# wangjunchi/LLMSeg

Hardware: AMD Instinct MI355X
Metric: images/sec (1024x1024, 64-tok prompt) model_forward fwd+bwd (higher is better)
Workload: dtype bf16; 1 GPU; BASELINE.json configs[2]: synthetic 1024x1024 + random-init LLaVA-7B(Llama-7B+CLIP-L/14)/SAM-ViT-H, batch_size=2 per GPU, fwd+bwd train step (CE + align + IoP losses, LoRA r=8 dropout 0.05 on q/v + trainable embed/lm_head/text_fcs/lisa_*, frozen towers, fp32 gradient arena, AdamW step every 10 micro-steps inside the timed region, micro-step replayed from a hipGraph), 256 candidate masks, 64-token ; global_batch=2, parallelism=dp1, graph=True, valid=True

## Files before the change

include/llmseg_hip.h:

```cpp
#ifndef LLMSEG_HIP_H
#define LLMSEG_HIP_H

#include <stdint.h>

#ifdef __cplusplus
extern "C" {
#endif

#define LLMSEG_OK 0
#define LLMSEG_EINVAL (-1)
#define LLMSEG_ELAUNCH (-2)
#define LLMSEG_NOT_TAKEN 1

enum { LLMSEG_ACT_NONE = 0, LLMSEG_ACT_RELU = 1, LLMSEG_ACT_GELU = 2, LLMSEG_ACT_QUICKGELU = 3, LLMSEG_ACT_SILU = 4,
       LLMSEG_ACT_SIGMOID = 5 };

#define LLMSEG_ABI_VERSION 11

#define LLMSEG_REDUCE_WS_BYTES (16 << 20)
int llmseg_version(void);
int64_t llmseg_launch_count(void);
int64_t llmseg_struct_size(int which);
const char* llmseg_last_error(void);

typedef struct {
  uint32_t struct_size;
  uint32_t reserved0;
  const void* A; const void* W; void* C;
  const void* bias;
  const void* gamma;
  const void* residual;
  int64_t M, N, K;
  int64_t lda, ldw, ldc, ldr;
  int64_t batch, strideA, strideW, strideC;
  float alpha;
  int act;
  int out_f32;
  int trans_a;
  int trans_w;
  int64_t batch2, strideA2, strideW2, strideC2;
// ... 137 lines not shown
int llmseg_intersection_union(const uint8_t* pred, const uint8_t* target, int64_t n, int32_t ignore_index, int64_t* out, void* stream);

int llmseg_union_resize_iou(const uint8_t* segs, const uint8_t* select, const uint8_t* gt, int32_t H, int32_t W, int32_t K, int32_t Hg, int32_t Wg,
                            int32_t out_h, int32_t out_w, int32_t ignore_index, int64_t* out, void* stream);

int llmseg_gt_resample(const uint8_t* gt, const int32_t* gy, const int32_t* gx, uint8_t* out, int32_t H, int32_t W, int32_t Hg, int32_t Wg, void* stream);
int llmseg_proposal_targets(const uint8_t* masks, const int64_t* order, const uint8_t* gtp, int32_t n_gt, void* out, int32_t K, int32_t H, int32_t W,
                            int32_t out_size, const int32_t* y0, const int32_t* ny, const double* wy, const int32_t* x0, const int32_t* nx,
                            const double* wx, int32_t taps, int64_t* counts, int64_t* gt_area, double* iou, double* iop, void* stream);
int llmseg_rle_decode(const uint32_t* run_ends, const int64_t* offsets, uint8_t* out, int32_t K, int32_t H, int32_t W, int32_t hwk, void* stream);
int llmseg_mask_targets(const uint8_t* segs, const uint8_t* gt, const int32_t* gy, const int32_t* gx, int32_t K, int32_t H, int32_t W, int32_t Hg,
                        int32_t Wg, int64_t* counts, int64_t* gt_area, double* iou, double* iop, void* stream);
int llmseg_resize_aa(const uint8_t* segs, void* out, int32_t K, int32_t H, int32_t W, int32_t out_size, const int32_t* y0, const int32_t* ny,
                     const double* wy, const int32_t* x0, const int32_t* nx, const double* wx, int32_t taps, void* stream);

int llmseg_colsum(const void* x, float* out, int64_t M, int64_t N, int64_t ld, void* workspace, int64_t workspace_bytes, void* stream);
int llmseg_norm_bwd(const void* dy, const void* x, const void* w, void* dx, float* dw, float* db, int64_t rows, int64_t cols,
                    float eps, int rms, void* workspace, int64_t workspace_bytes, void* stream);
int llmseg_norm_bwd_add(const void* dy, const void* x, const void* w, const void* dres, void* dx, float* dw, float* db, int64_t rows, int64_t cols,
                        float eps, int rms, void* workspace, int64_t workspace_bytes, void* stream);
int llmseg_swiglu_bwd(const void* gu, const void* dout, void* dgu, int64_t rows, int64_t I, void* stream);
int llmseg_act_bwd(const void* dy, const void* y, void* out, int64_t n, int act, void* stream);
int llmseg_linear_bwd(const void* dy, const void* y, int act, const void* x, const void* w, void* dx, float* dw, float* db, int64_t M, int64_t N, int64_t K,
                      int accumulate, void* stream);
int llmseg_softmax_rows(const float* S, void* P, int64_t BH, int32_t Tq, int32_t Tk, int32_t ld, float scale, int32_t causal,
                        const uint8_t* key_mask, int32_t heads, void* stream);
int llmseg_attn_ds(const void* P, const float* dP, void* dS, int64_t rows, int32_t T, int32_t ld, float scale, void* stream);
int llmseg_ce_bwd(const void* logits, const int64_t* labels, const float* coef, void* dlogits, int32_t N, int32_t T, int64_t V,
                  int64_t ldl, void* stream);
int llmseg_scatter_add_rows(const void* src, const int64_t* idx, float* dst, int64_t n, int64_t cols, void* stream);
typedef struct {
  const uint64_t* rng_state;
  uint32_t stream;
  uint32_t drop_thr;
  uint32_t seg_rows;
  uint32_t reserved0;
} llmseg_dropout;
int llmseg_lora_down(const void* x0, const void* x1, int64_t ldx, const void* w0, const void* w1, void* y, int64_t ldy, int64_t M, int64_t K,
                     int32_t w_kr, float alpha, int32_t zero_cols, const llmseg_dropout* drop, void* stream);
int llmseg_lora_down_ws(const void* x0, const void* x1, int64_t ldx, const void* w0, const void* w1, void* y, int64_t ldy, int64_t M, int64_t K,
                        int32_t w_kr, float alpha, int32_t zero_cols, const llmseg_dropout* drop, void* scratch, int64_t scratch_bytes, void* stream);
int llmseg_lora_outer(const void* a0, const void* a1, int64_t lda, const void* b0, const void* b1, int64_t ldb, float* out0, float* out1, int64_t M,
                      int64_t N, int32_t out_rn, float alpha, const llmseg_dropout* drop, void* workspace, int64_t workspace_bytes, void* stream);
int llmseg_lora_wgrads(const void* dq, const void* dv, int64_t ldd, const void* x, int64_t ldx, const void* xa, int64_t ldxa, const void* t, int64_t ldt,
                       float* gbq, float* gbv, float* gaq, float* gav, int64_t M, int64_t H, float s, const llmseg_dropout* drop, void* workspace,
                       int64_t workspace_bytes, void* stream);
int llmseg_lora_apply(void* y, int64_t ldy, const void* xa, int64_t ldxa, const void* w0, const void* w1, int64_t M, int64_t N, int32_t w_rn,
// ... 24 lines not shown
```

llmseg_amd/_lib.py:

```python
import ctypes as C
import os

_HERE = os.path.dirname(os.path.abspath(__file__))
LIB_PATH = os.environ.get("LLMSEG_LIB") or os.path.join(_HERE, "libllmseg_hip.so")

ABI_VERSION = 11

ACT_NONE, ACT_RELU, ACT_GELU, ACT_QUICKGELU, ACT_SILU, ACT_SIGMOID = range(6)
NOT_TAKEN = 1


class _Sized(C.Structure):

    def __init__(self, *a, **kw):
        super().__init__(*a, **kw)
        self.struct_size = C.sizeof(self)


class GemmArgs(_Sized):
    _fields_ = [("struct_size", C.c_uint32), ("reserved0", C.c_uint32), ("A", C.c_void_p), ("W", C.c_void_p), ("C", C.c_void_p),
                ("bias", C.c_void_p), ("gamma", C.c_void_p), ("residual", C.c_void_p),
                ("M", C.c_int64), ("N", C.c_int64), ("K", C.c_int64),
                ("lda", C.c_int64), ("ldw", C.c_int64), ("ldc", C.c_int64), ("ldr", C.c_int64),
                ("batch", C.c_int64), ("strideA", C.c_int64), ("strideW", C.c_int64), ("strideC", C.c_int64),
                ("alpha", C.c_float), ("act", C.c_int), ("out_f32", C.c_int), ("trans_a", C.c_int), ("trans_w", C.c_int),
                ("batch2", C.c_int64), ("strideA2", C.c_int64), ("strideW2", C.c_int64), ("strideC2", C.c_int64),
                ("A2", C.c_void_p), ("W2", C.c_void_p), ("lda2", C.c_int64), ("ldw2", C.c_int64),
                ("workspace", C.c_void_p), ("workspace_bytes", C.c_int64), ("accumulate", C.c_int),
                ("a_norm_w", C.c_void_p), ("a_norm_eps", C.c_float), ("a_swiglu", C.c_int),
# ... 77 lines not shown
    "llmseg_mask_pullback": [_p, _p, _p, _p, _i32, _i32, _i32, _p],
    "llmseg_upsample_maskpool": [_p, _p, _p, _p, _p, _p, _i32, _i32, _i32, _i32, _p],
    "llmseg_cosine_scores": [_p, _p, _p, _i32, _i32, _p],
    "llmseg_linear_f32": [_p, _i64, _p, _i64, _i32, _p, _p, _i64, _p, _i64, _i32, _i32, _i32, _i32, _f32, _p],
    "llmseg_layernorm_f32": [_p, _p, _p, _p, _i64, _i32, _f32, _p],
    "llmseg_attn_f32": [_p, _p, _p, _p, C.POINTER(C.c_int64), _i32, _i32, _i32, _i32, _i32, _f32, _p],
    "llmseg_cosine_f32": [_p, _p, _p, _i32, _i32, _p],
    "llmseg_align_reg_loss": [_p, _p, _p, _p, _p, _p, _p, _p, _p, _i32, _i32, _f32, _i32, _p],
    "llmseg_dice_bce": [_p, _p, _p, _i32, _i64, _f32, _p, _i64, _p],
    "llmseg_dice_bce_bwd": [_p, _p, _p, _p, _i32, _i64, _f32, _p],
    "llmseg_ce_loss": [_p, _p, _p, _i32, _i32, _i64, _i64, _p, _i64, _p],
    "llmseg_intersection_union": [_p, _p, _i64, _i32, _p, _p],
    "llmseg_union_resize_iou": [_p, _p, _p, _i32, _i32, _i32, _i32, _i32, _i32, _i32, _i32, _p, _p],
    "llmseg_rle_decode": [_p, _p, _p, _i32, _i32, _i32, _i32, _p],
    "llmseg_mask_targets": [_p, _p, _p, _p, _i32, _i32, _i32, _i32, _i32, _p, _p, _p, _p, _p],
    "llmseg_gt_resample": [_p, _p, _p, _p, _i32, _i32, _i32, _i32, _p],
    "llmseg_proposal_targets": [_p, _p, _p, _i32, _p, _i32, _i32, _i32, _i32, _p, _p, _p, _p, _p, _p, _i32, _p, _p, _p, _p, _p],
    "llmseg_resize_aa": [_p, _p, _i32, _i32, _i32, _i32, _p, _p, _p, _p, _p, _p, _i32, _p],
    "llmseg_colsum": [_p, _p, _i64, _i64, _i64, _p, _i64, _p],
    "llmseg_norm_bwd": [_p, _p, _p, _p, _p, _p, _i64, _i64, _f32, C.c_int, _p, _i64, _p],
    "llmseg_norm_bwd_add": [_p, _p, _p, _p, _p, _p, _p, _i64, _i64, _f32, C.c_int, _p, _i64, _p],
    "llmseg_swiglu_bwd": [_p, _p, _p, _i64, _i64, _p],
    "llmseg_act_bwd": [_p, _p, _p, _i64, C.c_int, _p],
    "llmseg_linear_bwd": [_p, _p, C.c_int, _p, _p, _p, _p, _p, _i64, _i64, _i64, C.c_int, _p],
    "llmseg_softmax_rows": [_p, _p, _i64, _i32, _i32, _i32, _f32, _i32, _p, _i32, _p],
    "llmseg_attn_ds": [_p, _p, _p, _i64, _i32, _i32, _f32, _p],
    "llmseg_ce_bwd": [_p, _p, _p, _p, _i32, _i32, _i64, _i64, _p],
    "llmseg_scatter_add_rows": [_p, _p, _p, _i64, _i64, _p],
    "llmseg_lora_down": [_p, _p, _i64, _p, _p, _p, _i64, _i64, _i64, _i32, _f32, _i32, _dp, _p],
    "llmseg_lora_down_ws": [_p, _p, _i64, _p, _p, _p, _i64, _i64, _i64, _i32, _f32, _i32, _dp, _p, _i64, _p],
    "llmseg_lora_outer": [_p, _p, _i64, _p, _p, _i64, _p, _p, _i64, _i64, _i32, _f32, _dp, _p, _i64, _p],
    "llmseg_lora_wgrads": [_p, _p, _i64, _p, _i64, _p, _i64, _p, _i64, _p, _p, _p, _p, _i64, _i64, _f32, _dp, _p, _i64, _p],
    "llmseg_lora_apply": [_p, _i64, _p, _i64, _p, _p, _i64, _i64, _i32, _f32, _dp, _p],
    "llmseg_lora_pack": [_p, _p, _p, _p, _p, _p, _p, _i64, _f32, _p],
    "llmseg_lora_down_parts": [_p, _p, _i64, _p, _p, _p, _i64, _i64, _i64, _i32, _f32, _i32, _dp, _p, _i64, C.POINTER(C.c_int32), C.POINTER(C.c_float), _p],
    "llmseg_lora_down_pack": [_p, _p, _i64, _p, _p, _p, _i64, _i64, _i64, _i32, _f32, _i32, _dp, _p, _i64, _p, _p, _p, _p, _p, _p, _p, _i64, _f32, _p],
    "llmseg_transpose_pad": [_p, _p, _i64, _i64, _i64, _i64, _i64, _p],
    "llmseg_sumsq": [_p, _i64, C.c_int, _p, _p, _i64, _p],
    "llmseg_adamw": [_p, _p, _p, C.c_int, _p, _p, _i64, _f32, _f32, _f32, _f32, _f32, _i64, _p, _p],
    "llmseg_prof_enable": [C.c_int],
    "llmseg_prof_dominant_kernel": [],
    "llmseg_prof_dominant_bytes": [],
    "llmseg_prof_dominant_info": [C.POINTER(C.c_int64)],
    "llmseg_prof_collect": [C.POINTER(C.c_double), C.POINTER(C.c_double), C.POINTER(C.c_int64), C.POINTER(C.c_double), C.POINTER(C.c_double),
                            C.POINTER(C.c_int64)],
}

# ... 30 lines not shown
```

llmseg_amd/autograd.py:

```python
import math
import os

import torch
from torch.autograd import Function

from . import ops

BF16 = torch.bfloat16


BIG_LINEAR = 1 << 34
BIG_WEIGHT = 1 << 26
FUSE_ROPE_BWD = os.environ.get("LLMSEG_NO_FUSE_ROPE_BWD") is None
FUSE_ROPE_FWD = os.environ.get("LLMSEG_NO_FUSE_ROPE_FWD") is None
FUSE_NORM_BWD = os.environ.get("LLMSEG_NO_FUSE_NORM_BWD") is None
FUSE_LORA_PARTS = os.environ.get("LLMSEG_NO_FUSE_LORA_PARTS") is None
FUSE_DELTA = os.environ.get("LLMSEG_NO_FUSE_DELTA") is None
FUSE_MLP = os.environ.get("LLMSEG_NO_FUSE_MLP") is None
FUSE_LINEAR_BWD = os.environ.get("LLMSEG_NO_FUSE_LINEAR_BWD") is None


class Leaves:
    on = False
    _streams = {}
    _keep = []
    _used = False

    @classmethod
    def run(cls, fn, *operands):
        if not cls.on:
            return fn()
        cur = torch.cuda.current_stream()
        key = cur.device.index
        side = cls._streams.get(key)
        if side is None:
            side = cls._streams[key] = torch.cuda.Stream(device=cur.device)
        side.wait_stream(cur)
        with torch.cuda.stream(side):
            out = fn()
        cls._keep.extend(operands)
        cls._used = True
        return out
# ... 26 lines not shown
    def forward(ctx, x, w, b, act, residual, wt=None):
        y = ops.gemm(x, w, bias=b, act=act, residual=residual)
        ctx.wt = wt
        ctx.act = act
        ctx.has_res = residual is not None
        ctx.gw, ctx.gb = g32_of(w), (g32_of(b) if b is not None else None)
        ctx.b_needs = b is not None and b.requires_grad
        assert not (act != ops.ACT_NONE and residual is not None)
        assert act in (ops.ACT_NONE, ops.ACT_RELU, ops.ACT_SIGMOID), "only relu/sigmoid epilogues are differentiated"
        ctx.save_for_backward(x, w, y if act != ops.ACT_NONE else None)
        return y

    @staticmethod
    def backward(ctx, dy):
        x, w, y = ctx.saved_tensors
        dy = dy.contiguous()
        N = w.shape[0]
        M, Kin = x.shape
        dx = dw = db = None
        gw = ctx.gw
        need_w = gw is not None or ctx.needs_input_grad[1]
        big = M * N * Kin >= BIG_LINEAR or (N * Kin >= BIG_WEIGHT and M >= 16)
        dres = dy if (ctx.has_res and ctx.needs_input_grad[4]) else None
        if FUSE_LINEAR_BWD and not Leaves.on and not (big and Kin % 8 == 0) and not (ctx.wt is not None and N % 8 == 0):
            need_b = ctx.gb is not None or (ctx.b_needs and ctx.needs_input_grad[2])
            acc = gw is not None or ctx.gb is not None
            new = torch.zeros if acc else torch.empty
            fw = gw if gw is not None else (new((N, Kin), device=x.device, dtype=torch.float32) if need_w else None)
            fb = ctx.gb if ctx.gb is not None else (new((N,), device=x.device, dtype=torch.float32) if need_b else None)
            if ctx.needs_input_grad[0] or fw is not None or fb is not None:
                r = ops.linear_bwd(dy, y, ctx.act, x.contiguous(), w.contiguous(), want_dx=ctx.needs_input_grad[0], dw=fw, db=fb, accumulate=acc)
                if not isinstance(r, str):
                    return (r, fw.to(BF16) if (gw is None and need_w) else None, fb.to(BF16) if (ctx.gb is None and need_b) else None, None, dres, None)
        dpre = ops.act_bwd(dy, y, ctx.act) if ctx.act != ops.ACT_NONE else dy
        if big and Kin % 8 == 0 and (need_w or ctx.wt is None or N % 8 != 0):
            Np, Mp = (N + 63) // 64 * 64, (M + 63) // 64 * 64
            if Np != N:
                dpp = torch.zeros((M, Np), device=dpre.device, dtype=BF16)
                dpp[:, :N] = dpre
            else:
                dpp = dpre
            if ctx.needs_input_grad[0]:
                dx = ops.gemm(dpp, ops.transpose_pad(w, Np))
            if need_w:
                if gw is not None:
                    def wgrad():
                        dT, xT = ops.transpose_pad(dpp, Mp), ops.transpose_pad(x, Mp)
                        ops.gemm(dT[:N], xT, out=gw, accumulate=True)
                    Leaves.run(wgrad, dpp, x)
                else:
                    dT, xT = ops.transpose_pad(dpp, Mp), ops.transpose_pad(x, Mp)
                    dw = ops.gemm(dT, xT)[:N]
        else:
            if N % 8 != 0:
                dpre_p = _pad8_cols(dpre)
                w_p = torch.zeros((dpre_p.shape[1], w.shape[1]), device=w.device, dtype=w.dtype)
                w_p[:N] = w
            else:
                dpre_p, w_p = dpre, w
            if ctx.needs_input_grad[0]:
                dx = ops.gemm(dpre, ctx.wt) if (ctx.wt is not None and N % 8 == 0) else ops.gemm(dpre_p, w_p, trans_w=True)
            if gw is not None:
                Leaves.run(lambda: ops.gemm(dpre_p[:, :N], x, out=gw, trans_a=True, trans_w=True, accumulate=True), dpre_p, x)
            elif need_w:
                dw = ops.gemm(dpre_p, x, trans_a=True, trans_w=True)[:N]
                if dw.shape[0] != N or not dw.is_contiguous():
                    dw = dw.contiguous()
        if ctx.gb is not None:
            Leaves.run(lambda: ops.colsum(dpre, out=ctx.gb), dpre)
        elif ctx.b_needs and ctx.needs_input_grad[2]:
            db = ops.colsum(dpre).to(BF16)
        return dx, dw, db, None, dres, None


def linear(x, w, b=None, act=ops.ACT_NONE, residual=None, wt=None):
    return LinearFn.apply(x, w, b, act, residual, wt)


class LinearNormFn(Function):

    @staticmethod
    def forward(ctx, x, w, b, act, residual, wt, norm_w, eps):
        assert b is None and act == ops.ACT_NONE and residual is not None
        h = torch.empty((x.shape[0], w.shape[0]), device=x.device, dtype=BF16)
        y = ops.gemm(x, w, residual=residual, norm_w=norm_w, norm_eps=eps, norm_out=h)
        ctx.wt, ctx.act, ctx.has_res = wt, act, True
        ctx.gw, ctx.gb, ctx.b_needs = g32_of(w), None, False
        ctx.save_for_backward(x, w, None)
        ctx.mark_non_differentiable(h)
        ctx.set_materialize_grads(False)
        return y, h

    @staticmethod
    def backward(ctx, dy, _dh):
        return LinearFn.backward(ctx, dy) + (None, None)


def linear_norm(x, w, residual, wt, norm_w, eps):
    return LinearNormFn.apply(x, w, None, ops.ACT_NONE, residual, wt, norm_w, eps)
# ... 557 lines not shown
```

llmseg_amd/csrc/backward.hip:

```cpp
#include <algorithm>
#include <cstdlib>
#include "common.h"
#include "llmseg_hip.h"

namespace {

inline unsigned grid_for(long total) {
  long g = (total + 255) / 256;
  return (unsigned)(g < 1 ? 1 : (g > 8192 ? 8192 : g));
}

__global__ __launch_bounds__(256) void colsum_kernel(const bf16_t* __restrict__ x, float* __restrict__ out, float* __restrict__ part, long M, long N, long ld) {
  __shared__ float red[4][64];
  const int c = threadIdx.x & 63, rl = threadIdx.x >> 6;
  const long col = (long)blockIdx.x * 64 + c;
  const long rows_per = (M + gridDim.y - 1) / gridDim.y;
  const long r0 = (long)blockIdx.y * rows_per, r1 = min(M, r0 + rows_per);
  float s = 0.f;
  if (col < N)
    for (long r = r0 + rl; r < r1; r += 4) s += bf2f(x[r * ld + col]);
  red[rl][c] = s;
  __syncthreads();
  if (rl == 0 && col < N) {
    const float v = (red[0][c] + red[1][c]) + (red[2][c] + red[3][c]);
// ... 1174 lines not shown
  const int rc = llmseg_lora_down_ws(x0, x1, ldx, w0, w1, y, ldy, M, K, w_kr, alpha, zero_cols, drop, scratch, scratch_bytes, stream);
  const bool done = g_pack_req.done;
  g_pack_req.active = false;
  if (rc != LLMSEG_OK || done) return rc;
  return llmseg_lora_pack(aq, bq, av, bv, w2b, w2a, bt, H, s, stream);
}

extern "C" int llmseg_transpose_pad(const void* in, void* out, int64_t rows, int64_t cols, int64_t ld_in, int64_t ld_out, int64_t rows_pad, void* stream) {
  LL_CHECK(in && out && rows > 0 && cols > 0 && rows_pad >= rows && ld_out >= rows_pad && ld_in >= cols, "transpose_pad: bad arguments");
  LL_CHECK((cols & 7) == 0 && (ld_in & 7) == 0 && (ld_out & 7) == 0 && (rows_pad & 7) == 0 && AL16(in) && AL16(out),
           "transpose_pad: cols, rows_pad and leading dimensions must be multiples of 8, pointers 16-byte aligned");
  LL_LAUNCH_KERNEL(transpose_pad_kernel, dim3((unsigned)((cols + 63) / 64), (unsigned)((rows_pad + 63) / 64)), dim3(256), 0, (hipStream_t)stream,
                     (const bf16_t*)in, (bf16_t*)out, (long)rows, (long)cols, (long)ld_in, (long)ld_out, (long)rows_pad);
  LL_LAUNCH_CHECK("transpose_pad");
  return LLMSEG_OK;
}

namespace {
constexpr int LB_TI = 32, LB_TK = 64, LB_CC = 256, LB_LD = LB_CC + 8;

struct LinBwd {
  const bf16_t *dy, *y, *x, *w;
  bf16_t* dx;
  float *dw, *db;
  int M, N, K, act, accumulate;
  int w_it, w_kt, x_kt;
  int vec_n, vec_k;
};

__device__ __forceinline__ uint4 lb_load8(const bf16_t* __restrict__ p, int r, int c, int rows, int cols, bool vec) {
  if (r >= rows || c >= cols) return make_uint4(0, 0, 0, 0);
  const bf16_t* q = p + (long)r * cols + c;
  if (vec) return *reinterpret_cast<const uint4*>(q);
  uint32_t h[8];
#pragma unroll
  for (int j = 0; j < 8; ++j) h[j] = c + j < cols ? (uint32_t)q[j] : 0u;
  return make_uint4(h[0] | (h[1] << 16), h[2] | (h[3] << 16), h[4] | (h[5] << 16), h[6] | (h[7] << 16));
}

__device__ __forceinline__ uint4 lb_act8(const uint4& g, const uint4& yv, int act) {
  if (act == LLMSEG_ACT_NONE) return g;
  float gf[8], yf[8];
  uint32_t o[8];
  unpack8(g, gf); unpack8(yv, yf);
#pragma unroll
  for (int e = 0; e < 8; ++e) o[e] = f2bf(act == LLMSEG_ACT_RELU ? (yf[e] > 0.f ? gf[e] : 0.f) : gf[e] * yf[e] * (1.f - yf[e]));
  return make_uint4(o[0] | (o[1] << 16), o[2] | (o[3] << 16), o[4] | (o[5] << 16), o[6] | (o[7] << 16));
}

__device__ __forceinline__ uint32_t lb_elem(const uint4& v, int j) {
  const uint32_t wd = (j >> 1) == 0 ? v.x : (j >> 1) == 1 ? v.y : (j >> 1) == 2 ? v.z : v.w;
  return (j & 1) ? (wd >> 16) : (wd & 0xffffu);
}

__device__ __forceinline__ void lb_store_t(bf16_t* T, int col0, int c, const uint4& lo, const uint4& hi) {
#pragma unroll
  for (int j = 0; j < 8; ++j) *reinterpret_cast<uint32_t*>(T + (col0 + j) * LB_LD + c) = lb_elem(lo, j) | (lb_elem(hi, j) << 16);
}

__global__ __launch_bounds__(256) void linear_bwd_kernel(const LinBwd p) {
  __shared__ __attribute__((aligned(16))) bf16_t lds[(LB_TI + LB_TK) * LB_LD];
  bf16_t* AT = lds;
  bf16_t* BT = lds + LB_TI * LB_LD;
  const int t = threadIdx.x, lane = t & 63, wave = t >> 6;
  const int nW = p.w_it * p.w_kt;
  const bool roleW = (int)blockIdx.x < nW;
  const int bi = roleW ? (int)blockIdx.x : (int)blockIdx.x - nW;
  const int nkt = roleW ? p.w_kt : p.x_kt;
  const int i0 = (bi / nkt) * LB_TI, k0 = (bi % nkt) * LB_TK;
  const int C = roleW ? p.M : p.N;
  const bf16_t* __restrict__ B = roleW ? p.x : p.w;
  const bool vn = p.vec_n != 0, vk = p.vec_k != 0, has_act = p.act != LLMSEG_ACT_NONE;
  const bool want_db = roleW && (bi % nkt) == 0 && p.db != nullptr;

  uint4 ra[4], ry[4], rb[8];
  auto load_chunk = [&](int c0) {
#pragma unroll
    for (int q = 0; q < 4; ++q) {
      int r, c;
      if (roleW) { const int pr = t + 256 * (q >> 1); r = c0 + 2 * (pr >> 2) + (q & 1); c = i0 + 8 * (pr & 3); }
      else { const int v = t + 256 * q; r = i0 + (v >> 5); c = c0 + 8 * (v & 31); }
      ra[q] = lb_load8(p.dy, r, c, p.M, p.N, vn);
      if (has_act) ry[q] = lb_load8(p.y, r, c, p.M, p.N, vn);
    }
#pragma unroll
    for (int q = 0; q < 8; ++q) {
      const int pr = t + 256 * (q >> 1);
      rb[q] = lb_load8(B, c0 + 2 * (pr >> 3) + (q & 1), k0 + 8 * (pr & 7), C, p.K, vk);
    }
  };
// ... 1 lines not shown
    if (has_act) {
#pragma unroll
      for (int q = 0; q < 4; ++q) ra[q] = lb_act8(ra[q], ry[q], p.act);
    }
    if (roleW) {
#pragma unroll
      for (int q = 0; q < 2; ++q) { const int pr = t + 256 * q; lb_store_t(AT, 8 * (pr & 3), 2 * (pr >> 2), ra[2 * q], ra[2 * q + 1]); }
    } else {
#pragma unroll
      for (int q = 0; q < 4; ++q) { const int v = t + 256 * q; *reinterpret_cast<uint4*>(AT + (v >> 5) * LB_LD + 8 * (v & 31)) = ra[q]; }
    }
#pragma unroll
    for (int q = 0; q < 4; ++q) { const int pr = t + 256 * q; lb_store_t(BT, 8 * (pr & 7), 2 * (pr >> 3), rb[2 * q], rb[2 * q + 1]); }
  };

  f32x4_t acc[2][4];
#pragma unroll
  for (int ib = 0; ib < 2; ++ib)
#pragma unroll
    for (int kb = 0; kb < 4; ++kb) acc[ib][kb] = f32x4_t{0.f, 0.f, 0.f, 0.f};
  float dbacc = 0.f;

  const int nch = (C + LB_CC - 1) / LB_CC;
  load_chunk(0);
  for (int ch = 0; ch < nch; ++ch) {
    if (ch) __syncthreads();
    store_chunk();
    __syncthreads();
    if (ch + 1 < nch) load_chunk((ch + 1) * LB_CC);
    if (want_db) {
      const bf16_t* row = AT + (t >> 3) * LB_LD + 32 * (t & 7);
#pragma unroll
      for (int v = 0; v < 4; ++v) {
        float f[8];
        unpack8(*reinterpret_cast<const uint4*>(row + 8 * v), f);
#pragma unroll
        for (int e = 0; e < 8; ++e) dbacc += f[e];
      }
    }
#pragma unroll
    for (int ks = 0; ks < 2; ++ks) {
      const int cw = wave * 64 + ks * 32;
      if (ch * LB_CC + cw >= C) break;
      const int cb = cw + 8 * (lane >> 4);
      bf16x8_t af[2], bf[4];
#pragma unroll
      for (int ib = 0; ib < 2; ++ib) af[ib] = *reinterpret_cast<const bf16x8_t*>(AT + (16 * ib + (lane & 15)) * LB_LD + cb);
#pragma unroll
      for (int kb = 0; kb < 4; ++kb) bf[kb] = *reinterpret_cast<const bf16x8_t*>(BT + (16 * kb + (lane & 15)) * LB_LD + cb);
#pragma unroll
      for (int ib = 0; ib < 2; ++ib)
#pragma unroll
// ... 11 lines not shown
  if (roleW && !p.dw) return;

  float* fold = reinterpret_cast<float*>(lds);
  __syncthreads();
#pragma unroll
  for (int ib = 0; ib < 2; ++ib)
#pragma unroll
    for (int kb = 0; kb < 4; ++kb)
#pragma unroll
      for (int e = 0; e < 4; ++e) fold[(wave * LB_TI + 16 * ib + 4 * (lane >> 4) + e) * LB_TK + 16 * kb + (lane & 15)] = acc[ib][kb][e];
  __syncthreads();
#pragma unroll
  for (int q = 0; q < 8; ++q) {
    const int idx = t + 256 * q, i = idx >> 6, k = idx & 63;
    float s = fold[idx];
    s += fold[LB_TI * LB_TK + idx];
    s += fold[2 * LB_TI * LB_TK + idx];
    s += fold[3 * LB_TI * LB_TK + idx];
    const int gi = i0 + i, gk = k0 + k;
    if (gk >= p.K) continue;
    if (roleW) {
      if (gi < p.N) { float* o = p.dw + (long)gi * p.K + gk; *o = p.accumulate ? *o + s : s; }
    } else if (gi < p.M) {
      p.dx[(long)gi * p.K + gk] = f2bf(s);
    }
  }
}
}

extern "C" int llmseg_linear_bwd(const void* dy, const void* y, int act, const void* x, const void* w, void* dx, float* dw, float* db, int64_t M, int64_t N, int64_t K,
                                 int accumulate, void* stream) {
  LL_CHECK(dy && x && w && M > 0 && N > 0 && K > 0 && (dx || dw || db), "linear_bwd: bad arguments");
  LL_CHECK(act == LLMSEG_ACT_NONE || ((act == LLMSEG_ACT_RELU || act == LLMSEG_ACT_SIGMOID) && y), "linear_bwd: only relu/sigmoid are differentiated, from the output y");
  if (M > 2048 || N * K > (1L << 22)) return LLMSEG_NOT_TAKEN;
  LinBwd p;
  p.dy = (const bf16_t*)dy; p.y = (const bf16_t*)y; p.x = (const bf16_t*)x; p.w = (const bf16_t*)w;
  p.dx = (bf16_t*)dx; p.dw = dw; p.db = db;
  p.M = (int)M; p.N = (int)N; p.K = (int)K; p.act = act; p.accumulate = accumulate ? 1 : 0;
  p.w_it = (dw || db) ? (int)((N + LB_TI - 1) / LB_TI) : 0;
  p.w_kt = dw ? (int)((K + LB_TK - 1) / LB_TK) : 1;
  p.x_kt = (int)((K + LB_TK - 1) / LB_TK);
  p.vec_n = (N & 7) == 0 && AL16(dy) && (act == LLMSEG_ACT_NONE || AL16(y));
  p.vec_k = (K & 7) == 0 && AL16(x) && AL16(w);
  const long grid = (long)p.w_it * p.w_kt + (dx ? (long)((M + LB_TI - 1) / LB_TI) * p.x_kt : 0L);
  LL_LAUNCH_KERNEL(linear_bwd_kernel, dim3((unsigned)grid), dim3(256), 0, (hipStream_t)stream, p);
  LL_LAUNCH_CHECK("linear_bwd");
  return LLMSEG_OK;
}
```

llmseg_amd/ops.py:

```python
import ctypes as C
import math

import torch

from . import _lib
from ._lib import (ACT_GELU, ACT_NONE, ACT_QUICKGELU, ACT_RELU, ACT_SIGMOID, ACT_SILU, AttnArgs, AttnBwdArgs, GemmArgs)

BF16 = torch.bfloat16


def _stream():
    return C.c_void_p(torch.cuda.current_stream().cuda_stream)


def _ptr(t):
    return None if t is None else C.c_void_p(t.data_ptr())


def _req(t, dtype=BF16):
    assert t.is_cuda and t.dtype == dtype, f"expected cuda {dtype}, got {t.device} {t.dtype}"
    return t


WS_BYTES = 192 << 20
# ... 534 lines not shown
def norm_bwd(dy, x, w, eps, rms, dw=None, db=None, dres=None, workspace=_DEFAULT_WS):
    rows, cols = x.shape
    assert dy.is_contiguous() and x.is_contiguous() and (dres is None or (dres.is_contiguous() and dres.shape == x.shape))
    dx = torch.empty_like(x)
    _lib.check(_lib.load().llmseg_norm_bwd_add(_ptr(dy), _ptr(x), _ptr(w), _ptr(dres), _ptr(dx), _ptr(dw), _ptr(db), rows, cols, eps, 1 if rms else 0,
                                               *_ws_arg(workspace, x.device), _stream()), "norm_bwd")
    return dx


def swiglu_bwd(gu, dout, inter):
    assert gu.is_contiguous() and dout.is_contiguous()
    dgu = torch.empty_like(gu)
    _lib.check(_lib.load().llmseg_swiglu_bwd(_ptr(gu), _ptr(dout), _ptr(dgu), gu.shape[0], inter, _stream()), "swiglu_bwd")
    return dgu


def act_bwd(dy, y, act):
    assert dy.is_contiguous() and y.is_contiguous()
    out = torch.empty_like(dy)
    _lib.check(_lib.load().llmseg_act_bwd(_ptr(dy), _ptr(y), _ptr(out), dy.numel(), act, _stream()), "act_bwd")
    return out


def linear_bwd(dy, y, act, x, w, want_dx=True, dw=None, db=None, accumulate=False, dx=None):
    M, N = dy.shape
    K = x.shape[1]
    _req(dy); _req(x); _req(w)
    assert dy.is_contiguous() and x.is_contiguous() and w.is_contiguous() and x.shape == (M, K) and w.shape == (N, K)
    assert act == ACT_NONE or (_req(y).is_contiguous() and y.shape == dy.shape)
    for g, shape in ((dw, (N, K)), (db, (N,))):
        assert g is None or (g.dtype == torch.float32 and g.is_contiguous() and g.shape == shape and g.is_cuda)
    if want_dx and dx is None:
        dx = torch.empty((M, K), device=dy.device, dtype=BF16)
    assert dx is None or (_req(dx).is_contiguous() and dx.shape == (M, K))
    rc = _lib.load().llmseg_linear_bwd(_ptr(dy), _ptr(y) if act != ACT_NONE else None, act, _ptr(x), _ptr(w), _ptr(dx), _ptr(dw), _ptr(db), M, N, K,
                                       1 if accumulate else 0, _stream())
    if rc == _lib.NOT_TAKEN:
        return "not taken"
    _lib.check(rc, "linear_bwd")
    return dx


def softmax_rows(S, BH, Tq, Tk, ld, scale, causal=False, key_mask=None, heads=1):
    P = torch.empty((BH, Tq, ld), device=S.device, dtype=BF16)
    _lib.check(_lib.load().llmseg_softmax_rows(_ptr(S), _ptr(P), BH, Tq, Tk, ld, scale, 1 if causal else 0, _ptr(key_mask), heads, _stream()),
               "softmax_rows")
    return P


def attn_ds(P, dP, T, ld, scale):
    dS = torch.empty_like(P)
    _lib.check(_lib.load().llmseg_attn_ds(_ptr(P), _ptr(dP), _ptr(dS), P.shape[0] * P.shape[1], T, ld, scale, _stream()), "attn_ds")
    return dS


def ce_bwd(logits, labels, coef, out=None):
    N, T, V = logits.shape
    ld = logits.stride(1)
    if out is not None:
# ... 183 lines not shown
```

llmseg_amd/trainable.py:

```python
import torch

from . import autograd as ag
from . import ops

IMAGE_TOKEN_INDEX = -200
IGNORE_INDEX = -100
BF16 = torch.bfloat16


class _Direct:
    grad = False
    linear = staticmethod(lambda x, w, b=None, act=ops.ACT_NONE, residual=None, wt=None: ops.gemm(x, w, bias=b, act=act, residual=residual))
    norm = staticmethod(lambda x, w, b=None, eps=1e-5, rms=False: ops.norm(x, w, b, eps=eps, rms=rms))
    norm_pass = staticmethod(lambda x, w, b=None, eps=1e-5, rms=False, pre=None: ((ops.norm(x, w, b, eps=eps, rms=rms) if pre is None else pre), x))

    @staticmethod
    def linear_norm(x, w, residual, wt, norm_w, eps):
        h = torch.empty((x.shape[0], w.shape[0]), device=x.device, dtype=BF16)
        return ops.gemm(x, w, residual=residual, norm_w=norm_w, norm_eps=eps, norm_out=h), h
    attn_packed = staticmethod(lambda qkv, batch, n, heads, hd, causal=False, key_mask=None:
                               ops.attention_packed(qkv, batch, n, heads, hd, causal=causal, key_mask=key_mask))
    swiglu = staticmethod(lambda gu, inter: ops.swiglu(gu, inter))
    embed_splice = staticmethod(lambda ids, emb, feats, P, fs, tok=None: ops.embed_splice(ids, emb, feats, P, feats_stride_n=fs))
    gather_rows = staticmethod(lambda x, idx: ops.gather_rows(x, idx))
    maskpool = staticmethod(lambda feat, segs, g, S: ops.upsample_maskpool(feat, segs, g, S))

    @staticmethod
    def rope_attn(qkv, rope, batch, n, heads, hd, causal, key_mask, pre_rotated=False):
        if not pre_rotated:
            ops.rope_(qkv, rope[0], rope[1], batch * n, n, 2 * heads, hd, qkv.stride(0))
        return ops.attention_packed(qkv, batch, n, heads, hd, causal=causal, key_mask=key_mask)

    @staticmethod
    def mlp(x, wgu, wgu_t, wd, wd_t, residual, norm_w, eps):
        M, inter = x.shape[0], wd.shape[1]
# ... 24 lines not shown
    @staticmethod
    def align_reg(e, t, pred, gt_iou, gt_iop):
        return ops.align_reg_loss(e, t, gt_iou, pred, gt_iop)

    @staticmethod
    def bcast_add(s, add, Cn, K):
        for ci in range(Cn):
            blk = s[ci * K:(ci + 1) * K]
            ops.add_rows(blk, add[ci:ci + 1].contiguous(), out=blk)
        return s

    @staticmethod
    def cross_attn_1q(q, kv, Cn, K, heads, hd):
        D = heads * hd
        o = torch.empty((Cn, D), device=q.device, dtype=BF16)
        ops.attention(q, kv, kv[:, D:], o, batch=Cn, heads=heads, Nq=1, Nk=K, head_dim=hd, q_strides=(D, hd, D),
                      k_strides=(K * 2 * D, hd, 2 * D), v_strides=(K * 2 * D, hd, 2 * D), o_strides=(D, hd, D))
        return o


class _Auto:
    grad = True
    linear = staticmethod(ag.linear)
    norm = staticmethod(ag.norm)
    norm_pass = staticmethod(ag.norm_pass)
    linear_norm = staticmethod(ag.linear_norm)
    attn_packed = staticmethod(lambda qkv, batch, n, heads, hd, causal=False, key_mask=None:
                               ag.PackedAttnFn.apply(qkv, batch, n, heads, hd, causal, key_mask, None))
    rope_attn = staticmethod(ag.rope_attention)
    swiglu = staticmethod(lambda gu, inter: ag.SwigluFn.apply(gu, inter))
    embed_splice = staticmethod(lambda ids, emb, feats, P, fs, tok=None: ag.EmbedSpliceFn.apply(ids, emb, feats, P, fs, tok))
    gather_rows = staticmethod(lambda x, idx: ag.GatherRowsFn.apply(x, idx))
    maskpool = staticmethod(lambda feat, segs, g, S: ag.MaskPoolFn.apply(feat, segs, g, S))
    lora_qkv = staticmethod(lambda x, wqkv, aq, bq, av, bv, s, wqkv_t=None, drop=None, rope=None:
                            ag.LoraQKVFn.apply(x, wqkv, aq, bq, av, bv, s, wqkv_t, drop, rope))
    mlp = staticmethod(ag.mlp)
    norm_lora_qkv = staticmethod(ag.norm_lora_qkv)
    norm_mlp = staticmethod(ag.norm_mlp)
    attn_oproj = staticmethod(ag.attn_oproj)
    ce = staticmethod(lambda logits, labels: ag.CELossFn.apply(logits, labels))
    align_reg = staticmethod(lambda e, t, pred, gt_iou, gt_iop: ag.AlignRegFn.apply(e, t, pred, gt_iou, gt_iop))
    bcast_add = staticmethod(lambda s, add, Cn, K: ag.BcastAddFn.apply(s, add, Cn, K))
    cross_attn_1q = staticmethod(lambda q, kv, Cn, K, heads, hd: ag.CrossAttn1QFn.apply(q, kv, Cn, K, heads, hd))


class BatchPlan:
# ... 275 lines not shown
        hidden = self._llama(embeds, plan.key_mask, F, drop_seg_rows=plan.__dict__.get("drop_seg_rows", 0))
        if F.grad and self.__dict__.get("_split_backward"):
            root, hidden = hidden, hidden.detach().requires_grad_(True)
            self.__dict__["_split_pair"] = (root, hidden)
        logits, loss = None, None
        gathered = plan.new_labels is not None and not want_logits and plan.ce_rows is not None and self.ce_gather_first
        if want_logits or (plan.new_labels is not None and not gathered):
            logits = F.linear(hidden.view(N * T, H), self._w("lm_head.weight", F)).view(N, T, -1)
        if gathered:
            rows = F.gather_rows(hidden.view(N * T, H), plan.ce_rows)
            lg = F.linear(rows, self._w("lm_head.weight", F)).view(1, rows.shape[0], -1)
            if plan.__dict__.get("micro", 1) > 1:
                loss = None
                for a, b in plan.ce_segs:
                    part = F.ce(lg[:, a:b], plan.ce_labels[:, a:b])
                    loss = part if loss is None else loss + part
            else:
                loss = F.ce(lg, plan.ce_labels)
        elif plan.new_labels is not None:
            assert plan.__dict__.get("micro", 1) == 1, "fused accumulation needs ce_gather_first (per-micro-batch CE segments)"
            loss = F.ce(logits, plan.new_labels)
        return loss, logits, hidden

    def _head_attn_1key(self, p, text, F):
        v = F.linear(text, self._w(p + "v_proj.weight", F), self._w(p + "v_proj.bias", F))
        return F.linear(v, self._w(p + "out_proj.weight", F), self._w(p + "out_proj.bias", F))

    def _ln(self, x, name, F):
        return F.norm(x, self._w(name + ".weight", F), self._w(name + ".bias", F), 1e-5, False)

    def _mask_head(self, pooled, text, F, stacked=False):
        Cn = text.shape[0]
        D = pooled.shape[1]
        K = pooled.shape[0] // Cn if stacked else pooled.shape[0]
        nh, hd = 8, D // 8
        if stacked:
            s = pooled
        else:
            s = pooled.repeat(Cn, 1) if Cn > 1 else (pooled.clone() if not F.grad else pooled)
        t = text.contiguous()
        trace = self.__dict__.get("_relu_trace")

        def lin(x, p, act=ops.ACT_NONE, res=None):
            y = F.linear(x, self._w(p + ".weight", F), self._w(p + ".bias", F), act, res)
            if trace is not None and act == ops.ACT_RELU:
                trace.setdefault(p, []).append(y.detach())
            return y
        for i in range(2):
            p = f"model.lisa_attention_layers.{i}."
            w, b = self._qkv_wb(p + "self_attn.", F)
            a = F.attn_packed(F.linear(s, w, b), Cn, K, nh, hd)
            s = self._ln(lin(a, p + "self_attn.out_proj", res=s), p + "norm1", F)
            s = self._ln(F.bcast_add(s, self._head_attn_1key(p + "cross_attn_token_to_image.", t, F), Cn, K), p + "norm2", F)
            s = self._ln(lin(lin(s, p + "mlp.lin1", ops.ACT_RELU), p + "mlp.lin2", res=s), p + "norm3", F)
            pc = p + "cross_attn_image_to_token."
            q = lin(t, pc + "q_proj")
            kvw, kvb = self._kv_wb(pc, F, D)
            kv = F.linear(s, kvw, kvb)
            o = F.cross_attn_1q(q, kv, Cn, K, nh, hd)
            t = self._ln(lin(o, pc + "out_proj", res=t), p + "norm4", F)
        s = self._ln(F.bcast_add(s, self._head_attn_1key("model.lisa_final_attn.", t, F), Cn, K), "model.lisa_norm_final_attn", F)
        iou = lin(lin(s, "model.lisa_iou_head.0", ops.ACT_RELU), "model.lisa_iou_head.2", ops.ACT_SIGMOID)
        emb = lin(lin(s, "model.lisa_embedding_head.0", ops.ACT_RELU), "model.lisa_embedding_head.2")
        return iou.view(Cn * K), emb

    def _mask_head_f32(self, pooled, text):
        P = self.params
        Cn, (K, D) = text.shape[0], pooled.shape
        nh, hd = 8, D // 8
        s = pooled.repeat(Cn, 1) if Cn > 1 else pooled
        t = text.contiguous()
        lin = lambda x, p, act=ops.ACT_NONE, res=None: ops.linear_f32(x, P[p + ".weight"], P[p + ".bias"], act, res)
        ln = lambda x, p: ops.layernorm_f32(x, P[p + ".weight"], P[p + ".bias"], 1e-5)
        one_key = lambda p, tt: lin(lin(tt, p + "v_proj"), p + "out_proj")
        bcast = lambda ss, add: (ss.view(Cn, K, D) + add[:, None, :]).view(Cn * K, D)
        for i in range(2):
            p = f"model.lisa_attention_layers.{i}."
            qkv = ops.linear_f32(s, P[p + "self_attn.qkv.weight"], P[p + "self_attn.qkv.bias"])
            a = torch.empty((Cn * K, D), device=s.device, dtype=torch.float32)
            st = (K * 3 * D, hd, 3 * D)
            ops.attention_f32(qkv, qkv[:, D:], qkv[:, 2 * D:], a, Cn, nh, K, K, hd, st, st, st, (K * D, hd, D))
            s = ln(lin(a, p + "self_attn.out_proj", res=s), p + "norm1")
            s = ln(bcast(s, one_key(p + "cross_attn_token_to_image.", t)), p + "norm2")
            s = ln(lin(lin(s, p + "mlp.lin1", ops.ACT_RELU), p + "mlp.lin2", res=s), p + "norm3")
            pc = p + "cross_attn_image_to_token."
# ... 209 lines not shown
```

Baseline: 52.63 images/s.

## Fuse residual-branch gradient add into linear backward and split-K dx slices

Adds a linear_tap autograd op that returns the input alongside the output, so the gradient from the other consumer of that input is added inside the fused linear backward kernel instead of by a separate autograd accumulation. The mask-head linears whose inputs fan out are rewritten to use it. The fused linear_bwd kernel also gains dx slicing across the reduction dimension, with fp32 partials in workspace and a fold kernel, which raises the size limit so larger weights take the fused path. This removes extra elementwise adds and separate launches, at the cost of workspace traffic and one extra fold launch when slicing is used.

```diff
diff --git a/include/llmseg_hip.h b/include/llmseg_hip.h
--- a/include/llmseg_hip.h
+++ b/include/llmseg_hip.h
@@ -15,7 +15,7 @@
 enum { LLMSEG_ACT_NONE = 0, LLMSEG_ACT_RELU = 1, LLMSEG_ACT_GELU = 2, LLMSEG_ACT_QUICKGELU = 3, LLMSEG_ACT_SILU = 4,
        LLMSEG_ACT_SIGMOID = 5 };
 
-#define LLMSEG_ABI_VERSION 11
+#define LLMSEG_ABI_VERSION 12
 
 #define LLMSEG_REDUCE_WS_BYTES (16 << 20)
 int llmseg_version(void);
@@ -199,7 +199,7 @@
 int llmseg_swiglu_bwd(const void* gu, const void* dout, void* dgu, int64_t rows, int64_t I, void* stream);
 int llmseg_act_bwd(const void* dy, const void* y, void* out, int64_t n, int act, void* stream);
 int llmseg_linear_bwd(const void* dy, const void* y, int act, const void* x, const void* w, void* dx, float* dw, float* db, int64_t M, int64_t N, int64_t K,
-                      int accumulate, void* stream);
+                      int accumulate, const void* dres, int64_t ld_dres, int dx_slices, void* workspace, int64_t workspace_bytes, void* stream);
 int llmseg_softmax_rows(const float* S, void* P, int64_t BH, int32_t Tq, int32_t Tk, int32_t ld, float scale, int32_t causal,
                         const uint8_t* key_mask, int32_t heads, void* stream);
 int llmseg_attn_ds(const void* P, const float* dP, void* dS, int64_t rows, int32_t T, int32_t ld, float scale, void* stream);
diff --git a/llmseg_amd/_lib.py b/llmseg_amd/_lib.py
--- a/llmseg_amd/_lib.py
+++ b/llmseg_amd/_lib.py
@@ -4,7 +4,7 @@
 _HERE = os.path.dirname(os.path.abspath(__file__))
 LIB_PATH = os.environ.get("LLMSEG_LIB") or os.path.join(_HERE, "libllmseg_hip.so")
 
-ABI_VERSION = 11
+ABI_VERSION = 12
 
 ACT_NONE, ACT_RELU, ACT_GELU, ACT_QUICKGELU, ACT_SILU, ACT_SIGMOID = range(6)
 NOT_TAKEN = 1
@@ -128,7 +128,7 @@
     "llmseg_norm_bwd_add": [_p, _p, _p, _p, _p, _p, _p, _i64, _i64, _f32, C.c_int, _p, _i64, _p],
     "llmseg_swiglu_bwd": [_p, _p, _p, _i64, _i64, _p],
     "llmseg_act_bwd": [_p, _p, _p, _i64, C.c_int, _p],
-    "llmseg_linear_bwd": [_p, _p, C.c_int, _p, _p, _p, _p, _p, _i64, _i64, _i64, C.c_int, _p],
+    "llmseg_linear_bwd": [_p, _p, C.c_int, _p, _p, _p, _p, _p, _i64, _i64, _i64, C.c_int, _p, _i64, C.c_int, _p, _i64, _p],
     "llmseg_softmax_rows": [_p, _p, _i64, _i32, _i32, _i32, _f32, _i32, _p, _i32, _p],
     "llmseg_attn_ds": [_p, _p, _p, _i64, _i32, _i32, _f32, _p],
     "llmseg_ce_bwd": [_p, _p, _p, _p, _i32, _i32, _i64, _i64, _p],
diff --git a/llmseg_amd/autograd.py b/llmseg_amd/autograd.py
--- a/llmseg_amd/autograd.py
+++ b/llmseg_amd/autograd.py
@@ -18,6 +18,8 @@
 FUSE_DELTA = os.environ.get("LLMSEG_NO_FUSE_DELTA") is None
 FUSE_MLP = os.environ.get("LLMSEG_NO_FUSE_MLP") is None
 FUSE_LINEAR_BWD = os.environ.get("LLMSEG_NO_FUSE_LINEAR_BWD") is None
+FUSE_DRES = os.environ.get("LLMSEG_NO_FUSE_DRES") is None
+LINEAR_BWD_SPLIT = os.environ.get("LLMSEG_NO_LINEAR_BWD_SPLIT") is None
 
 
 class Leaves:
@@ -90,6 +92,7 @@
         need_w = gw is not None or ctx.needs_input_grad[1]
         big = M * N * Kin >= BIG_LINEAR or (N * Kin >= BIG_WEIGHT and M >= 16)
         dres = dy if (ctx.has_res and ctx.needs_input_grad[4]) else None
+        dtap = getattr(ctx, "dtap", None) if ctx.needs_input_grad[0] else None
         if FUSE_LINEAR_BWD and not Leaves.on and not (big and Kin % 8 == 0) and not (ctx.wt is not None and N % 8 == 0):
             need_b = ctx.gb is not None or (ctx.b_needs and ctx.needs_input_grad[2])
             acc = gw is not None or ctx.gb is not None
@@ -97,7 +100,9 @@
             fw = gw if gw is not None else (new((N, Kin), device=x.device, dtype=torch.float32) if need_w else None)
             fb = ctx.gb if ctx.gb is not None else (new((N,), device=x.device, dtype=torch.float32) if need_b else None)
             if ctx.needs_input_grad[0] or fw is not None or fb is not None:
-                r = ops.linear_bwd(dy, y, ctx.act, x.contiguous(), w.contiguous(), want_dx=ctx.needs_input_grad[0], dw=fw, db=fb, accumulate=acc)
+                r = ops.linear_bwd(dy, y, ctx.act, x.contiguous(), w.contiguous(), want_dx=ctx.needs_input_grad[0], dw=fw, db=fb, accumulate=acc,
+                                   dres=None if dtap is None else dtap.contiguous(),
+                                   workspace=ops._DEFAULT_WS if LINEAR_BWD_SPLIT else None)
                 if not isinstance(r, str):
                     return (r, fw.to(BF16) if (gw is None and need_w) else None, fb.to(BF16) if (ctx.gb is None and need_b) else None, None, dres, None)
         dpre = ops.act_bwd(dy, y, ctx.act) if ctx.act != ops.ACT_NONE else dy
@@ -138,11 +143,37 @@
             Leaves.run(lambda: ops.colsum(dpre, out=ctx.gb), dpre)
         elif ctx.b_needs and ctx.needs_input_grad[2]:
             db = ops.colsum(dpre).to(BF16)
+        if dtap is not None:
+            dx = dx + dtap
         return dx, dw, db, None, dres, None
 
 
 def linear(x, w, b=None, act=ops.ACT_NONE, residual=None, wt=None):
     return LinearFn.apply(x, w, b, act, residual, wt)
+
+
+class LinearTapFn(Function):
+
+    @staticmethod
+    def forward(ctx, x, w, b, act):
+        y = LinearFn.forward(ctx, x, w, b, act, None)
+        ctx.set_materialize_grads(False)
+        if not ctx.needs_input_grad[0]:
+            ctx.mark_non_differentiable(x)
+        return y, x
+
+    @staticmethod
+    def backward(ctx, dy, dtap):
+        if dy is None:
+            return dtap, None, None, None
+        ctx.dtap = dtap
+        return LinearFn.backward(ctx, dy)[:4]
+
+
+def linear_tap(x, w, b=None, act=ops.ACT_NONE):
+    if not FUSE_DRES:
+        return linear(x, w, b, act), x
+    return LinearTapFn.apply(x, w, b, act)
 
 
 class LinearNormFn(Function):
diff --git a/llmseg_amd/csrc/backward.hip b/llmseg_amd/csrc/backward.hip
--- a/llmseg_amd/csrc/backward.hip
+++ b/llmseg_amd/csrc/backward.hip
@@ -1220,9 +1220,11 @@
 struct LinBwd {
   const bf16_t *dy, *y, *x, *w;
   bf16_t* dx;
+  const bf16_t* dres;
   float *dw, *db;
-  int M, N, K, act, accumulate;
-  int w_it, w_kt, x_kt;
+  float* part;
+  int M, N, K, act, accumulate, ld_dres;
+  int w_it, w_kt, x_kt, x_sl;
   int vec_n, vec_k;
 };
 
@@ -1263,7 +1265,9 @@
   const int t = threadIdx.x, lane = t & 63, wave = t >> 6;
   const int nW = p.w_it * p.w_kt;
   const bool roleW = (int)blockIdx.x < nW;
-  const int bi = roleW ? (int)blockIdx.x : (int)blockIdx.x - nW;
+  const int xb = (int)blockIdx.x - nW;
+  const int bi = roleW ? (int)blockIdx.x : xb / p.x_sl;
+  const int sl = roleW ? 0 : xb % p.x_sl;
   const int nkt = roleW ? p.w_kt : p.x_kt;
   const int i0 = (bi / nkt) * LB_TI, k0 = (bi % nkt) * LB_TK;
   const int C = roleW ? p.M : p.N;
@@ -1311,12 +1315,14 @@
   float dbacc = 0.f;
 
   const int nch = (C + LB_CC - 1) / LB_CC;
-  load_chunk(0);
-  for (int ch = 0; ch < nch; ++ch) {
-    if (ch) __syncthreads();
+  const int nsl = roleW ? 1 : p.x_sl;
+  const int ch0 = (int)((long)sl * nch / nsl), ch1 = (int)((long)(sl + 1) * nch / nsl);
+  load_chunk(ch0 * LB_CC);
+  for (int ch = ch0; ch < ch1; ++ch) {
+    if (ch != ch0) __syncthreads();
     store_chunk();
     __syncthreads();
-    if (ch + 1 < nch) load_chunk((ch + 1) * LB_CC);
+    if (ch + 1 < ch1) load_chunk((ch + 1) * LB_CC);
     if (want_db) {
       const bf16_t* row = AT + (t >> 3) * LB_LD + 32 * (t & 7);
 #pragma unroll
@@ -1374,28 +1380,58 @@
     if (roleW) {
       if (gi < p.N) { float* o = p.dw + (long)gi * p.K + gk; *o = p.accumulate ? *o + s : s; }
     } else if (gi < p.M) {
+      if (p.x_sl > 1) { p.part[((long)sl * p.M + gi) * p.K + gk] = s; continue; }
+      if (p.dres) s += bf2f(p.dres[(long)gi * p.ld_dres + gk]);
       p.dx[(long)gi * p.K + gk] = f2bf(s);
     }
   }
 }
+
+__global__ __launch_bounds__(256) void linear_bwd_fold_dx_kernel(const float* __restrict__ part, int P, long n, int K, const bf16_t* dres, long ld_dres, bf16_t* dx) {
+  for (long i = (long)blockIdx.x * blockDim.x + threadIdx.x; i < n; i += (long)gridDim.x * blockDim.x) {
+    float s = 0.f;
+    for (int q = 0; q < P; ++q) s += part[(long)q * n + i];
+    if (dres) s += bf2f(dres[(i / K) * ld_dres + i % K]);
+    dx[i] = f2bf(s);
+  }
+}
 }
 
 extern "C" int llmseg_linear_bwd(const void* dy, const void* y, int act, const void* x, const void* w, void* dx, float* dw, float* db, int64_t M, int64_t N, int64_t K,
-                                 int accumulate, void* stream) {
+                                 int accumulate, const void* dres, int64_t ld_dres, int dx_slices, void* workspace, int64_t workspace_bytes, void* stream) {
   LL_CHECK(dy && x && w && M > 0 && N > 0 && K > 0 && (dx || dw || db), "linear_bwd: bad arguments");
   LL_CHECK(act == LLMSEG_ACT_NONE || ((act == LLMSEG_ACT_RELU || act == LLMSEG_ACT_SIGMOID) && y), "linear_bwd: only relu/sigmoid are differentiated, from the output y");
-  if (M > 2048 || N * K > (1L << 22)) return LLMSEG_NOT_TAKEN;
+  LL_CHECK(!dres || (dx && ld_dres >= K && (dres != dx || ld_dres == K)), "linear_bwd: dres needs dx, a row pitch >= K, and dx's pitch when it is dx itself");
+  LL_CHECK(dx_slices >= 0, "linear_bwd: dx_slices < 0");
+  if (M > 2048 || N * K > (1L << 24)) return LLMSEG_NOT_TAKEN;
+  const int nch = (int)((N + LB_CC - 1) / LB_CC);
+  const long x_it = (M + LB_TI - 1) / LB_TI, x_kt = (K + LB_TK - 1) / LB_TK;
+  long sl = 1;
+  if (dx) {
+    if (dx_slices > 0) sl = dx_slices;
+    else if (N * K > (1L << 22)) sl = std::max(1L, 1024 / (x_it * x_kt));
+    sl = std::min(sl, (long)nch);
+  }
+  const int64_t need = sl > 1 ? sl * M * K * (int64_t)sizeof(float) : 0;
+  if (N * K > (1L << 22) && dx && sl <= 1) return LLMSEG_NOT_TAKEN;
+  if (need && (!workspace || workspace_bytes < need || !AL16(workspace))) {
+    if (dx_slices > 0) { llmseg_set_error("linear_bwd: %ld slices need %ld bytes of workspace", sl, (long)need); return LLMSEG_EINVAL; }
+    return LLMSEG_NOT_TAKEN;
+  }
   LinBwd p;
   p.dy = (const bf16_t*)dy; p.y = (const bf16_t*)y; p.x = (const bf16_t*)x; p.w = (const bf16_t*)w;
-  p.dx = (bf16_t*)dx; p.dw = dw; p.db = db;
-  p.M = (int)M; p.N = (int)N; p.K = (int)K; p.act = act; p.accumulate = accumulate ? 1 : 0;
+  p.dx = (bf16_t*)dx; p.dres = (const bf16_t*)dres; p.dw = dw; p.db = db; p.part = (float*)workspace;
+  p.M = (int)M; p.N = (int)N; p.K = (int)K; p.act = act; p.accumulate = accumulate ? 1 : 0; p.ld_dres = (int)ld_dres;
   p.w_it = (dw || db) ? (int)((N + LB_TI - 1) / LB_TI) : 0;
   p.w_kt = dw ? (int)((K + LB_TK - 1) / LB_TK) : 1;
-  p.x_kt = (int)((K + LB_TK - 1) / LB_TK);
+  p.x_kt = (int)x_kt; p.x_sl = (int)sl;
   p.vec_n = (N & 7) == 0 && AL16(dy) && (act == LLMSEG_ACT_NONE || AL16(y));
   p.vec_k = (K & 7) == 0 && AL16(x) && AL16(w);
-  const long grid = (long)p.w_it * p.w_kt + (dx ? (long)((M + LB_TI - 1) / LB_TI) * p.x_kt : 0L);
+  const long grid = (long)p.w_it * p.w_kt + (dx ? x_it * x_kt * sl : 0L);
   LL_LAUNCH_KERNEL(linear_bwd_kernel, dim3((unsigned)grid), dim3(256), 0, (hipStream_t)stream, p);
+  if (sl > 1)
+    LL_LAUNCH_KERNEL(linear_bwd_fold_dx_kernel, dim3(fold_grid(M * K)), dim3(256), 0, (hipStream_t)stream, (const float*)workspace, (int)sl, (long)(M * K), (int)K,
+                     (const bf16_t*)dres, (long)ld_dres, (bf16_t*)dx);
   LL_LAUNCH_CHECK("linear_bwd");
   return LLMSEG_OK;
 }
diff --git a/llmseg_amd/ops.py b/llmseg_amd/ops.py
--- a/llmseg_amd/ops.py
+++ b/llmseg_amd/ops.py
@@ -580,7 +580,7 @@
     return out
 
 
-def linear_bwd(dy, y, act, x, w, want_dx=True, dw=None, db=None, accumulate=False, dx=None):
+def linear_bwd(dy, y, act, x, w, want_dx=True, dw=None, db=None, accumulate=False, dx=None, dres=None, dx_slices=0, workspace=None):
     M, N = dy.shape
     K = x.shape[1]
     _req(dy); _req(x); _req(w)
@@ -591,8 +591,10 @@
     if want_dx and dx is None:
         dx = torch.empty((M, K), device=dy.device, dtype=BF16)
     assert dx is None or (_req(dx).is_contiguous() and dx.shape == (M, K))
+    assert dres is None or (dx is not None and _req(dres).shape == (M, K) and dres.stride(1) == 1 and (M == 1 or dres.stride(0) >= K))
     rc = _lib.load().llmseg_linear_bwd(_ptr(dy), _ptr(y) if act != ACT_NONE else None, act, _ptr(x), _ptr(w), _ptr(dx), _ptr(dw), _ptr(db), M, N, K,
-                                       1 if accumulate else 0, _stream())
+                                       1 if accumulate else 0, _ptr(dres), (max(dres.stride(0), K) if M > 1 else K) if dres is not None else 0, dx_slices,
+                                       *_ws_arg(workspace, dy.device), _stream())
     if rc == _lib.NOT_TAKEN:
         return "not taken"
     _lib.check(rc, "linear_bwd")
diff --git a/llmseg_amd/trainable.py b/llmseg_amd/trainable.py
--- a/llmseg_amd/trainable.py
+++ b/llmseg_amd/trainable.py
@@ -11,6 +11,7 @@
 class _Direct:
     grad = False
     linear = staticmethod(lambda x, w, b=None, act=ops.ACT_NONE, residual=None, wt=None: ops.gemm(x, w, bias=b, act=act, residual=residual))
+    linear_tap = staticmethod(lambda x, w, b=None, act=ops.ACT_NONE: (ops.gemm(x, w, bias=b, act=act), x))
     norm = staticmethod(lambda x, w, b=None, eps=1e-5, rms=False: ops.norm(x, w, b, eps=eps, rms=rms))
     norm_pass = staticmethod(lambda x, w, b=None, eps=1e-5, rms=False, pre=None: ((ops.norm(x, w, b, eps=eps, rms=rms) if pre is None else pre), x))
 
@@ -81,6 +82,7 @@
 class _Auto:
     grad = True
     linear = staticmethod(ag.linear)
+    linear_tap = staticmethod(ag.linear_tap)
     norm = staticmethod(ag.norm)
     norm_pass = staticmethod(ag.norm_pass)
     linear_norm = staticmethod(ag.linear_norm)
@@ -402,9 +404,13 @@
             loss = F.ce(logits, plan.new_labels)
         return loss, logits, hidden
 
-    def _head_attn_1key(self, p, text, F):
-        v = F.linear(text, self._w(p + "v_proj.weight", F), self._w(p + "v_proj.bias", F))
-        return F.linear(v, self._w(p + "out_proj.weight", F), self._w(p + "out_proj.bias", F))
+    def _head_attn_1key(self, p, text, F, tap=False):
+        if tap:
+            v, text = F.linear_tap(text, self._w(p + "v_proj.weight", F), self._w(p + "v_proj.bias", F))
+        else:
+            v = F.linear(text, self._w(p + "v_proj.weight", F), self._w(p + "v_proj.bias", F))
+        o = F.linear(v, self._w(p + "out_proj.weight", F), self._w(p + "out_proj.bias", F))
+        return (o, text) if tap else o
 
     def _ln(self, x, name, F):
         return F.norm(x, self._w(name + ".weight", F), self._w(name + ".bias", F), 1e-5, False)
@@ -426,21 +432,31 @@
             if trace is not None and act == ops.ACT_RELU:
                 trace.setdefault(p, []).append(y.detach())
             return y
+
+        def tap(x, p, act=ops.ACT_NONE):
+            y, x = F.linear_tap(x, self._w(p + ".weight", F), self._w(p + ".bias", F), act)
+            if trace is not None and act == ops.ACT_RELU:
+                trace.setdefault(p, []).append(y.detach())
+            return y, x
         for i in range(2):
             p = f"model.lisa_attention_layers.{i}."
             w, b = self._qkv_wb(p + "self_attn.", F)
-            a = F.attn_packed(F.linear(s, w, b), Cn, K, nh, hd)
+            qkv, s = F.linear_tap(s, w, b)
+            a = F.attn_packed(qkv, Cn, K, nh, hd)
             s = self._ln(lin(a, p + "self_attn.out_proj", res=s), p + "norm1", F)
-            s = self._ln(F.bcast_add(s, self._head_attn_1key(p + "cross_attn_token_to_image.", t, F), Cn, K), p + "norm2", F)
-            s = self._ln(lin(lin(s, p + "mlp.lin1", ops.ACT_RELU), p + "mlp.lin2", res=s), p + "norm3", F)
+            o, t = self._head_attn_1key(p + "cross_attn_token_to_image.", t, F, tap=True)
+            s = self._ln(F.bcast_add(s, o, Cn, K), p + "norm2", F)
+            h, s = tap(s, p + "mlp.lin1", ops.ACT_RELU)
+            s = self._ln(lin(h, p + "mlp.lin2", res=s), p + "norm3", F)
             pc = p + "cross_attn_image_to_token."
-            q = lin(t, pc + "q_proj")
+            q, t = tap(t, pc + "q_proj")
             kvw, kvb = self._kv_wb(pc, F, D)
-            kv = F.linear(s, kvw, kvb)
+            kv, s = F.linear_tap(s, kvw, kvb)
             o = F.cross_attn_1q(q, kv, Cn, K, nh, hd)
             t = self._ln(lin(o, pc + "out_proj", res=t), p + "norm4", F)
         s = self._ln(F.bcast_add(s, self._head_attn_1key("model.lisa_final_attn.", t, F), Cn, K), "model.lisa_norm_final_attn", F)
-        iou = lin(lin(s, "model.lisa_iou_head.0", ops.ACT_RELU), "model.lisa_iou_head.2", ops.ACT_SIGMOID)
+        h, s = tap(s, "model.lisa_iou_head.0", ops.ACT_RELU)
+        iou = lin(h, "model.lisa_iou_head.2", ops.ACT_SIGMOID)
         emb = lin(lin(s, "model.lisa_embedding_head.0", ops.ACT_RELU), "model.lisa_embedding_head.2")
         return iou.view(Cn * K), emb
 
```

After: 52.57 images/s. About the same (-0.1%).
